# baycom/tfrec

Measured on AMD Instinct MI355X. Metric: IQ MSamples/s through demod+decode (batched streams), higher is better.
Workload: dtype int32+f32+f64

## Files before the change

### tfrec_amd/csrc/chains2.hip

```cpp
#include <stdlib.h>

#include <algorithm>

#include "decoder_dev.h"
#include <type_traits>
#include "whb_chain_asm.h"

namespace tfrec {

constexpr int kSpecLbi = -(1 << 30);

__device__ __forceinline__ int whb_hook_perturb(const WinTables &T)
{
#ifdef TFREC_AMD_EXPERIMENTS
	return T.whb_test_perturb;
#else
	return 0;
#endif
}
__device__ __forceinline__ int whb_hook_force_fail(const WinTables &T)
{
#ifdef TFREC_AMD_EXPERIMENTS
	return T.whb_force_fail;
#else
	return 0;
#endif
}

__device__ __forceinline__ int tfa1_decay(int m) { return m - (int)(((uint32_t)m + 19u) / 20u); }

constexpr int kStatTfa1Scalar = 7, kStatTfa2Scalar = 8, kStatTfa1Vector = 9, kStatTfa2Vector = 10;
struct GroupStats {
	int scalar, vector;
};
__device__ __forceinline__ void stat_flush(const WinTables &T, const GroupStats &g, int slot_scalar, int slot_vector)
{
#if !defined(TFREC_AMD_COOPSTAT) && !defined(TFREC_AMD_VECSTAT) && !defined(TFREC_AMD_PROFILE_WHB)
	if ((threadIdx.x & 63) == 0) {
		if (g.scalar)
			atomicAdd(&T.stats[slot_scalar], (unsigned long long)g.scalar);
#ifdef TFREC_AMD_EXPERIMENTS
		if (g.vector)
			atomicAdd(&T.stats[slot_vector], (unsigned long long)g.vector);
#endif
	}
#endif
}

__device__ __forceinline__ int rebase_lbi(int lbi, int from_block, int to_block)
{
	return lbi ? lbi - kIndexSpan * (to_block - from_block) : 0;
}

struct BitWriter {
	uint32_t *base;
	uint32_t acc;
	int n;
	uint32_t pend;
	int pend_idx;
	__device__ __forceinline__ void put(int bit)
	{
		acc |= (uint32_t)bit << (n & 31);
		n++;
		if ((n & 31) == 0) {
			if (pend_idx >= 0)
				base[pend_idx] = pend;
			pend = acc;
			pend_idx = (n >> 5) - 1;
			acc = 0;
		}
	}
	__device__ __forceinline__ void put_bits(uint32_t v, int cnt)
	{
		const int sh = n & 31;
		const unsigned long long a = (unsigned long long)acc | ((unsigned long long)v << sh);
		n += cnt;
		if (sh + cnt >= 32) {
			if (pend_idx >= 0)
				base[pend_idx] = pend;
			pend = (uint32_t)a;
			pend_idx = (n >> 5) - 1;
			acc = (uint32_t)(a >> 32);
		} else {
			acc = (uint32_t)a;
		}
	}
	__device__ __forceinline__ void chunk_end()
	{
		const int idx = pend_idx >= 0 ? pend_idx : (n >> 5);
		base[idx] = pend_idx >= 0 ? pend : acc;
		pend_idx = -1;
	}
	__device__ __forceinline__ void finish()
	{
		chunk_end();
		if (n & 31)
			base[n >> 5] = acc;
	}
};

#include "windows.h"

#include "biquad.h"

#include "slicers.h"

#include "coop_slicer.h"

#include "whb_commit.h"

#include "whb_demod.h"

#include "whb_check.h"

#include "decode.h"

hipError_t launch_fmdev(hipStream_t st, const uint32_t *dec, size_t dec_stride, const unsigned long long *mask,
			size_t mask_stride, const uint32_t *prevdec, int16_t *fmdev, size_t fmdev_stride, EventBuf *eb,
			int n_streams, int n_blocks, int wmax, double flag_eps);

hipError_t launch_pipeline(const PipeCtl &P, const uint32_t *dec, size_t dec_stride, const unsigned long long *mask,
			   size_t mask_stride, const int16_t *fmdev, size_t fmdev_stride, int n_streams, int n_blocks,
			   long long sample_base, const ChainLaunch &L, const WinTables &T, int16_t *ld16, int32_t *dev32,
			   tfrec_amd_event *events, EventBuf *eb, uint32_t flags)
{
	auto mark = [&](int k, hipStream_t s_) {
		if (P.tev)
			(void)hipEventRecord(P.tev[k], s_);
	};
	hipError_t e = hipSuccess;
#define TRY(x)                          \
	do {                            \
		if ((e = (x)) != hipSuccess) \
			return e;       \
	} while (0)
	if (L.n_active == 0) {
		for (int k = 0; k < 3; k++)
			TRY(hipEventRecord(P.done[k], k == 0 ? P.cs : (k == 1 ? P.aux : P.t1)));
		return hipSuccess;
	}
	constexpr int lanes = 64;
	constexpr int head_chunks = 64;
	dim3 block(64);
	dim3 grid((n_streams + lanes - 1) / lanes, L.n_active);
	const int win_blocks = std::min(16384, (int)(((size_t)n_streams * n_blocks * 2 + lanes - 1) / lanes));
	const int seg_blocks = std::min(16384, (int)(((size_t)L.n_active * n_streams * ((size_t)n_blocks * (kBlockDec / 32) / kSegSlots + 4) +
						       lanes - 1) / lanes));
	const int repair_blocks = std::min(seg_blocks, std::max(256, seg_blocks / 8));
	const int spec_blocks = std::min(seg_blocks, std::max(256, seg_blocks / 5));
	const int long_window = (size_t)n_streams * L.n_active >= 1024 ? kLongWindow : kLongWindow / 2;
	const int coop_blocks = std::min(32768, std::max(1, (int)std::min<size_t>((size_t)L.n_active * n_streams *
								((size_t)n_blocks * kBlockDec / (size_t)long_window + 1), 1u << 30)));
	const int dec_blocks = std::min(16384, std::max(1, win_blocks));
	bool has_whb = false, has_tfa2 = false, has_tfa1 = false;
	for (int a = 0; a < L.n_active; a++) {
		has_whb = has_whb || L.params[a].kind == 2;
		has_tfa2 = has_tfa2 || L.params[a].kind == 1;
		has_tfa1 = has_tfa1 || L.params[a].kind == 0;
	}
// ... 147 lines not shown
```

### tfrec_amd/csrc/whb_check.h

```cpp
#pragma once

#ifndef TFREC_AMD_CHK_STREAMS
#define TFREC_AMD_CHK_STREAMS 32
#endif
constexpr int kChkStreams = TFREC_AMD_CHK_STREAMS;
constexpr int kChkProducers = 2;
constexpr int kChkPerProducer = kChkStreams / kChkProducers;
static_assert(kChkStreams <= 64 && kChkStreams % kChkProducers == 0, "a lane per stream, the streams split evenly");
constexpr int kChkPairRow = 64 * 4 + 4;
constexpr int kChkDevRow = 64 + 4;
struct ChkBuf {
	uint32_t pair[kChkStreams * kChkPairRow];
	uint32_t dev[kChkStreams * kChkDevRow];
};
constexpr size_t kChkLdsBytes = 2 * sizeof(ChkBuf);

__global__ __launch_bounds__(64 * (1 + kChkProducers)) void whb_chain_kernel(int n_streams, ChainLaunch L, int a, WinTables T)
{
	extern __shared__ __attribute__((aligned(16))) uint8_t chk_lds[];
	ChkBuf *const buf = reinterpret_cast<ChkBuf *>(chk_lds);
	const int wave = (int)threadIdx.x >> 6, ln = (int)threadIdx.x & 63;
	const int s0 = (int)blockIdx.x * kChkStreams;
	const ChainParams &p = L.params[a];
	const double a1 = p.iir_avg.a1, a2 = p.iir_avg.a2, bh = 0.5 * p.iir_avg.b0;
	const int my_s = s0 + ln;
	const bool my_on = ln < kChkStreams && my_s < n_streams;
	const int my_rounds = my_on ? T.whbdense_n[my_s] >> 6 : 0;
	int rmax = my_rounds;
#pragma unroll
	for (int o = 32; o >= 1; o >>= 1) {
		const int other = __shfl_xor(rmax, o, 64);
		rmax = other > rmax ? other : rmax;
	}
	rmax = __builtin_amdgcn_readfirstlane(rmax);
	if (rmax == 0)
		return;
	if (wave == 0) {
		double y1 = 0.0, y2 = 0.0;
		if (my_on) {
			const WhbExact st = T.whbx[my_s];
			y1 = st.y1;
			y2 = st.y2;
		}
		unsigned long long *const xbits = T.whbxbits + (size_t)(my_on ? my_s : 0) * T.whbx_stride;
		double2 *const xsnap = T.whbxsnap + (size_t)(my_on ? my_s : 0) * T.whbx_stride;
		__syncthreads();
		for (int r = 0; r < rmax; r++) {
			if (r < my_rounds) {
				const ChkBuf &b = buf[r & 1];
				const double2 *prow = reinterpret_cast<const double2 *>(b.pair + ln * kChkPairRow);
				const uint4 *drow = reinterpret_cast<const uint4 *>(b.dev + ln * kChkDevRow);
				uint32_t acc[2] = { 0u, 0u };
				double2 pq[2][8];
				uint4 dq[2][2];
				auto fetch = [&](int h, int g8) {
#pragma unroll
					for (int j = 0; j < 8; j++)
						pq[h][j] = prow[8 * g8 + j];
					dq[h][0] = drow[2 * g8];
					dq[h][1] = drow[2 * g8 + 1];
				};
				fetch(0, 0);
#pragma unroll
				for (int g8 = 0; g8 < 8; g8++) {
					const int h = g8 & 1;
					if (g8 + 1 < 8)
						fetch(h ^ 1, g8 + 1);
					const int dv[8] = { (int)dq[h][0].x, (int)dq[h][0].y, (int)dq[h][0].z, (int)dq[h][0].w,
							    (int)dq[h][1].x, (int)dq[h][1].y, (int)dq[h][1].z, (int)dq[h][1].w };
#pragma unroll
					for (int j = 0; j < 8; j++) {
						const double P = pq[h][j].x, B2 = pq[h][j].y;
						const double y = ((B2 + a1 * y1) + P) + a2 * y2;
						y2 = y1;
						y1 = y;
						const int yi = (int)y;
						asm("v_cmp_lt_i32 vcc, %1, %2\n\tv_addc_co_u32 %0, vcc, %0, %0, vcc" : "+v"(acc[g8 >> 2]) : "v"(dv[j]), "v"(yi) : "vcc");
					}
				}
				xbits[r] = (unsigned long long)__brev(acc[0]) | ((unsigned long long)__brev(acc[1]) << 32);
				xsnap[r] = make_double2(y1, y2);
			}
			__syncthreads();
		}
	} else {
		const int q0 = (wave - 1) * kChkPerProducer;
		int rounds[kChkPerProducer], h1[kChkPerProducer], h2[kChkPerProducer];
		const int32_t *row[kChkPerProducer];
#pragma unroll
		for (int q = 0; q < kChkPerProducer; q++) {
			const int s = s0 + q0 + q;
			const bool on = s < n_streams;
			rounds[q] = __builtin_amdgcn_readlane(my_rounds, (q0 + q) & 63);
			row[q] = T.whbdense + (size_t)(on ? s : 0) * T.whbdense_stride;
			const WhbExact st = T.whbx[on ? s : 0];
			h1[q] = __builtin_amdgcn_readfirstlane(st.fd1);
			h2[q] = __builtin_amdgcn_readfirstlane(st.fd2);
		}
		int cur[kChkPerProducer], nxt[kChkPerProducer];
#pragma unroll
		for (int q = 0; q < kChkPerProducer; q++) {
			cur[q] = rounds[q] > 0 ? row[q][ln] : 0;
			nxt[q] = rounds[q] > 1 ? row[q][64 + ln] : 0;
		}
		auto lay_out = [&](ChkBuf &b, int r) {
#pragma unroll
			for (int q = 0; q < kChkPerProducer; q++) {
				if (r < rounds[q]) {
					const int d0 = cur[q];
					const int s1 = __builtin_amdgcn_update_dpp(0, d0, 0x138, 0xf, 0xf, false);
					const int d1 = ln == 0 ? h1[q] : s1;
					const int s2 = __builtin_amdgcn_update_dpp(0, d1, 0x138, 0xf, 0xf, false);
					const int d2 = ln == 0 ? h2[q] : s2;
					const double t0 = bh * (double)d0, t1 = bh * (double)d1, t2 = bh * (double)d2;
					const double P = __builtin_fma(2.0, t1, t0);
					*reinterpret_cast<double2 *>(b.pair + (q0 + q) * kChkPairRow + 4 * ln) = make_double2(P, t2);
					b.dev[(q0 + q) * kChkDevRow + ln] = (uint32_t)d0;
					h1[q] = __builtin_amdgcn_readlane(d0, 63);
					h2[q] = __builtin_amdgcn_readlane(d0, 62);
				}
			}
		};
		lay_out(buf[0], 0);
		__syncthreads();
		for (int r = 0; r < rmax; r++) {
			int far[kChkPerProducer];
#pragma unroll
			for (int q = 0; q < kChkPerProducer; q++)
				far[q] = r + 2 < rounds[q] ? row[q][64 * (r + 2) + ln] : 0;
#pragma unroll
			for (int q = 0; q < kChkPerProducer; q++)
				cur[q] = nxt[q];
			if (r + 1 < rmax)
				lay_out(buf[(r + 1) & 1], r + 1);
#pragma unroll
			for (int q = 0; q < kChkPerProducer; q++)
				nxt[q] = far[q];
			__syncthreads();
		}
	}
}

constexpr int kChkLockCap = 256;
__global__ __launch_bounds__(64) void whb_check_kernel(int n_streams, ChainLaunch L, int a, WinTables T, int *__restrict__ carry_io)
{
	__shared__ int lk_pos[kChkLockCap], lk_avgf[kChkLockCap];
	__shared__ uint32_t lk_meta[kChkLockCap];
	const int s = (int)blockIdx.x, ln = (int)threadIdx.x;
	if (s >= n_streams)
		return;
	const ChainParams &p = L.params[a];
	const double a1 = p.iir_avg.a1, a2 = p.iir_avg.a2, bh = 0.5 * p.iir_avg.b0;
	const int N = T.whbdense_n[s], R = N >> 6;
	const int32_t *dense = T.whbdense + (size_t)s * T.whbdense_stride;
	const unsigned long long *xbits = T.whbxbits + (size_t)s * T.whbx_stride;
	const double2 *xsnap = T.whbxsnap + (size_t)s * T.whbx_stride;
	const WhbExact st0 = T.whbx[s];
	const int tp_ = whb_hook_perturb(T);
	const int tol = tp_ > 1 ? tp_ : (tp_ < -1 ? -tp_ : 1);
	auto input = [&](int pos) -> int { return pos >= 0 ? dense[pos] : (pos == -1 ? st0.fd1 : st0.fd2); };
	auto run = [&](int rr, int cnt, double &y1, double &y2, unsigned long long &bits) {
		const int p0 = 64 * rr;
		if (rr == 0) {
			y1 = st0.y1;
			y2 = st0.y2;
		} else {
			const double2 sn = xsnap[rr - 1];
			y1 = sn.x;
			y2 = sn.y;
		}
		double t1 = bh * (double)input(p0 - 1), t2 = bh * (double)input(p0 - 2);
		bits = 0ull;
		for (int k = 0; k < cnt; k++) {
			const int d = dense[p0 + k];
			const double t0 = bh * (double)d;
			const double P = __builtin_fma(2.0, t1, t0);
			const double y = ((t2 + a1 * y1) + P) + a2 * y2;
			bits |= (unsigned long long)(d < (int)y ? 1u : 0u) << k;
			y2 = y1;
			y1 = y;
			t2 = t1;
			t1 = t0;
		}
	};
	double yf1 = 0.0, yf2 = 0.0;
	unsigned long long tailbits = 0ull;
	if (ln == 0)
		run(R, N & 63, yf1, yf2, tailbits);
	tailbits = __shfl(tailbits, 0, 64);
	auto word = [&](int i) -> unsigned long long { return i < R ? xbits[i] : (i == R ? tailbits : 0ull); };
	const uint4 *recrow = reinterpret_cast<const uint4 *>(T.whbrec + (size_t)s * T.whbrec_stride);
	int carry = carry_io[s];
	const int carry_in = carry;
	bool bad = false;
	int cbase = 0, nlocks = 0;
	bool ended = false;
	int last_delta = 0;
	bool have_last = false, last_closed = false;
	auto do_locks = [&]() {
		for (int b0 = 0; b0 < nlocks; b0 += 64) {
			const int i = b0 + ln;
			const bool on = i < nlocks;
			double y1 = 0.0, y2 = 0.0;
			unsigned long long bits;
			const int pos = on ? lk_pos[i] : 0;
			run(pos >> 6, on ? (pos & 63) + 1 : 0, y1, y2, bits);
			const uint32_t meta = on ? lk_meta[i] : 0u;
			const int delta = (int)y1 - (on ? lk_avgf[i] : 0);
			const bool b = on && (delta > tol || delta < -tol || (delta != 0 && (meta & kWhbRecAmb)));
			bad = bad || __ballot(b) != 0ull;
			const int nb = nlocks - b0 < 64 ? nlocks - b0 : 64;
			last_delta = __shfl(delta, nb - 1, 64);
			last_closed = (__shfl((int)meta, nb - 1, 64) & (int)kWhbRecClosed) != 0;
			have_last = true;
		}
		nlocks = 0;
	};
	for (int v0 = 0; !ended; v0 += 64) {
		const int vi = v0 + ln < T.whbrec_stride - 1 ? v0 + ln : T.whbrec_stride - 1;
		const uint4 rec = recrow[vi];
		const uint32_t meta = rec.z;
		const unsigned long long endm = __ballot(meta == kWhbRecEnd);
		const int nrec = endm ? __builtin_ctzll(endm) : 64;
		ended = endm != 0ull || v0 + 64 + 64 > T.whbrec_stride;
		const bool on = ln < nrec;
		const bool pseudo = on && (meta & kWhbRecPseudo) != 0u;
		const bool normal = on && !pseudo;
		const int nv = normal ? (int)((meta >> kWhbRecNvShift) & 63u) + 1 : 0;
		int inc = nv;
#pragma unroll
		for (int o = 1; o < 64; o <<= 1) {
			const int up = __shfl_up(inc, o, 64);
			inc += ln >= o ? up : 0;
		}
		const int pos0 = cbase + inc - nv;
		cbase += __shfl(inc, 63, 64);
		if (pseudo) {
			if (v0 + ln == 0) {
				bad = bad || (carry != 0 && (meta & kWhbRecAmb));
				if (meta & kWhbRecClosed)
					carry = 0;
			} else {
				bad = true;
			}
		}
		if (normal) {
			const int w = pos0 >> 6, sh = pos0 & 63;
			const unsigned long long lo = word(w) >> sh, hi = sh ? word(w + 1) << (64 - sh) : 0ull;
			const unsigned long long vm = nv >= 64 ? ~0ull : (1ull << nv) - 1ull;
			const unsigned long long below = ((unsigned long long)rec.y << 32) | rec.x;
			bad = bad || (((lo | hi) ^ below) & vm) != 0ull || pos0 + nv > N;
		}
		carry = __shfl(carry, 0, 64);
		const bool lock = normal && (meta & kWhbRecLock) != 0u;
		const unsigned long long lm = __ballot(lock);
		if (lm) {
			if (nlocks + 64 > kChkLockCap)
				do_locks();
			if (lock) {
				const int i = nlocks + __builtin_popcountll(lm & ((1ull << ln) - 1ull));
				lk_pos[i] = pos0 + nv - 1;
				lk_avgf[i] = (int)rec.w;
				lk_meta[i] = meta;
			}
			nlocks += __builtin_popcountll(lm);
			__syncthreads();
		}
	}
	if (nlocks)
		do_locks();
	bad = __ballot(bad) != 0ull || cbase != N;
	if (have_last)
		carry = last_closed ? 0 : last_delta;
	if (ln == 0) {
		WhbExact st = st0;
		st.carry = carry_in;
		st.pad_ = 0;
		T.whbx0[s] = st;
		bad = bad || T.whbseen[s] != T.whbgen[s];
		if (whb_hook_force_fail(T) > 0 && (s + T.whb_submit_seq) % whb_hook_force_fail(T) == 0)
			bad = true;
		st.y1 = yf1;
		st.y2 = yf2;
		st.fd1 = input(N - 1);
		st.fd2 = input(N - 2);
		st.carry = st.pad_ = 0;
		T.whbx[s] = st;
		carry_io[s] = bad ? 0 : carry;
		T.whbfail[s] = bad ? 1 : 0;
	}
}

// ... 1 lines not shown
```

Measured before the change: 303,600.

## Move IIR threshold decisions to producer waves and hand-schedule consumer recurrence in asm

The consumer wave now runs only the serial f64 IIR recurrence through a generated inline-asm block with explicit LDS read lookahead, and writes each y value back to LDS. The compare-against-sample bit packing and the xbits/xsnap global stores move to the producer waves, which use ballots one round behind. The intent is to shorten the serial critical path on the consumer wave by taking the integer conversion, compare and global stores off it. In exchange, LDS traffic grows with the y row, the asm hardcodes VGPRs 64-105, and the producers gain a decide stage and an extra drain step.

```diff
diff --git a/tfrec_amd/csrc/chains2.hip b/tfrec_amd/csrc/chains2.hip
--- a/tfrec_amd/csrc/chains2.hip
+++ b/tfrec_amd/csrc/chains2.hip
@@ -5,6 +5,7 @@
 #include "decoder_dev.h"
 #include <type_traits>
 #include "whb_chain_asm.h"
+#include "whb_consumer_asm.h"
 
 namespace tfrec {
 
diff --git a/tfrec_amd/csrc/gen_whb_consumer.py b/tfrec_amd/csrc/gen_whb_consumer.py
--- /dev/null
+++ b/tfrec_amd/csrc/gen_whb_consumer.py
@@ -0,0 +1,85 @@
+#!/usr/bin/env python3
+import os
+import sys
+
+BASE = 64
+LOOKAHEAD = 8
+N_IN = 64
+REG_PAIR = [BASE + 4 * i for i in range(LOOKAHEAD)]
+REG_T = BASE + 4 * LOOKAHEAD
+REG_Q = [REG_T + 2, REG_T + 4]
+REG_Y01 = [REG_T + 6, REG_T + 8]
+LAST = REG_T + 9
+
+
+def vp(r):
+    return "v[%d:%d]" % (r, r + 1)
+
+
+def y(k):
+    k &= 3
+    return vp(REG_Y01[k]) if k < 2 else "%%[Y%d]" % k
+
+
+def pair_p(k):
+    return vp(REG_PAIR[k % LOOKAHEAD])
+
+
+def pair_b(k):
+    return vp(REG_PAIR[k % LOOKAHEAD] + 2)
+
+
+def block():
+    L = []
+    lgkm = []
+
+    def read(k):
+        L.append("ds_read_b128 v[%d:%d], %%[prow] offset:%d" % (REG_PAIR[k % LOOKAHEAD], REG_PAIR[k % LOOKAHEAD] + 3, 16 * k))
+        lgkm.append(("r", k))
+
+    def write(k):
+        L.append("ds_write2_b64 %%[yrow], %s, %s offset0:%d offset1:%d" % (y(k), y(k + 1), k, k + 1))
+        lgkm.append(("w", k))
+
+    def wait_for(op):
+        n = len(lgkm) - 1 - lgkm.index(op)
+        L.append("s_waitcnt lgkmcnt(%d)" % min(n, 15))
+
+    for k in range(LOOKAHEAD):
+        read(k)
+    L.append("v_mul_f64 %s, %%[a2], %s" % (vp(REG_Q[0]), y(-2)))
+    for k in range(N_IN):
+        L.append("v_mul_f64 %s, %%[a1], %s" % (vp(REG_T), y(k - 1)))
+        if k + 1 < N_IN:
+            L.append("v_mul_f64 %s, %%[a2], %s" % (vp(REG_Q[(k + 1) & 1]), y(k - 1)))
+        if k % 2 == 0:
+            wait_for(("r", k + 1))
+        L.append("v_add_f64 %s, %s, %s" % (vp(REG_T), pair_b(k), vp(REG_T)))
+        if k % 2 == 0 and k >= 2:
+            write(k - 2)
+        L.append("v_add_f64 %s, %s, %s" % (vp(REG_T), vp(REG_T), pair_p(k)))
+        if k + LOOKAHEAD < N_IN:
+            read(k + LOOKAHEAD)
+        L.append("v_add_f64 %s, %s, %s" % (y(k), vp(REG_T), vp(REG_Q[k & 1])))
+    write(N_IN - 2)
+    L.append("s_waitcnt lgkmcnt(0)")
+    return L
+
+
+def header():
+    out = ["// GENERATED by tfrec_amd/csrc/gen_whb_consumer.py -- do not edit (see the generator for the design).", "#pragma once",
+           "#define TFREC_WHB_CONSUMER_ASM \\"]
+    out.append(" \\\n".join('\t"%s\\n"' % x for x in block()))
+    out.append("#define TFREC_WHB_CONSUMER_CLOBBERS %s" % ", ".join('"v%d"' % r for r in range(BASE, LAST + 1)))
+    return "\n".join(out) + "\n"
+
+
+def main():
+    out = sys.argv[1] if len(sys.argv) > 1 else os.path.join(os.path.dirname(os.path.abspath(__file__)), "whb_consumer_asm.h")
+    with open(out, "w") as f:
+        f.write(header())
+    print("wrote", out)
+
+
+if __name__ == "__main__":
+    main()
diff --git a/tfrec_amd/csrc/whb_check.h b/tfrec_amd/csrc/whb_check.h
--- a/tfrec_amd/csrc/whb_check.h
+++ b/tfrec_amd/csrc/whb_check.h
@@ -8,12 +8,18 @@
 constexpr int kChkPerProducer = kChkStreams / kChkProducers;
 static_assert(kChkStreams <= 64 && kChkStreams % kChkProducers == 0, "a lane per stream, the streams split evenly");
 constexpr int kChkPairRow = 64 * 4 + 4;
-constexpr int kChkDevRow = 64 + 4;
+constexpr int kChkYRow = 64 * 2 + 4;
 struct ChkBuf {
 	uint32_t pair[kChkStreams * kChkPairRow];
-	uint32_t dev[kChkStreams * kChkDevRow];
+	uint32_t y[kChkStreams * kChkYRow];
 };
 constexpr size_t kChkLdsBytes = 2 * sizeof(ChkBuf);
+static_assert(kChkLdsBytes <= 160 * 1024, "one workgroup per CU");
+
+__device__ inline uint32_t chk_lds_addr(const uint32_t *p)
+{
+	return (uint32_t)(uintptr_t)(const __attribute__((address_space(3))) uint32_t *)p;
+}
 
 __global__ __launch_bounds__(64 * (1 + kChkProducers)) void whb_chain_kernel(int n_streams, ChainLaunch L, int a, WinTables T)
 {
@@ -42,44 +48,16 @@
 			y1 = st.y1;
 			y2 = st.y2;
 		}
-		unsigned long long *const xbits = T.whbxbits + (size_t)(my_on ? my_s : 0) * T.whbx_stride;
-		double2 *const xsnap = T.whbxsnap + (size_t)(my_on ? my_s : 0) * T.whbx_stride;
+		const int row = ln < kChkStreams ? ln : 0;
 		__syncthreads();
 		for (int r = 0; r < rmax; r++) {
 			if (r < my_rounds) {
 				const ChkBuf &b = buf[r & 1];
-				const double2 *prow = reinterpret_cast<const double2 *>(b.pair + ln * kChkPairRow);
-				const uint4 *drow = reinterpret_cast<const uint4 *>(b.dev + ln * kChkDevRow);
-				uint32_t acc[2] = { 0u, 0u };
-				double2 pq[2][8];
-				uint4 dq[2][2];
-				auto fetch = [&](int h, int g8) {
-#pragma unroll
-					for (int j = 0; j < 8; j++)
-						pq[h][j] = prow[8 * g8 + j];
-					dq[h][0] = drow[2 * g8];
-					dq[h][1] = drow[2 * g8 + 1];
-				};
-				fetch(0, 0);
-#pragma unroll
-				for (int g8 = 0; g8 < 8; g8++) {
-					const int h = g8 & 1;
-					if (g8 + 1 < 8)
-						fetch(h ^ 1, g8 + 1);
-					const int dv[8] = { (int)dq[h][0].x, (int)dq[h][0].y, (int)dq[h][0].z, (int)dq[h][0].w,
-							    (int)dq[h][1].x, (int)dq[h][1].y, (int)dq[h][1].z, (int)dq[h][1].w };
-#pragma unroll
-					for (int j = 0; j < 8; j++) {
-						const double P = pq[h][j].x, B2 = pq[h][j].y;
-						const double y = ((B2 + a1 * y1) + P) + a2 * y2;
-						y2 = y1;
-						y1 = y;
-						const int yi = (int)y;
-						asm("v_cmp_lt_i32 vcc, %1, %2\n\tv_addc_co_u32 %0, vcc, %0, %0, vcc" : "+v"(acc[g8 >> 2]) : "v"(dv[j]), "v"(yi) : "vcc");
-					}
-				}
-				xbits[r] = (unsigned long long)__brev(acc[0]) | ((unsigned long long)__brev(acc[1]) << 32);
-				xsnap[r] = make_double2(y1, y2);
+				const uint32_t prow = chk_lds_addr(b.pair + row * kChkPairRow), yrow = chk_lds_addr(b.y + row * kChkYRow);
+				asm volatile(TFREC_WHB_CONSUMER_ASM
+					     : [Y2] "+v"(y2), [Y3] "+v"(y1)
+					     : [prow] "v"(prow), [yrow] "v"(yrow), [a1] "s"(a1), [a2] "s"(a2)
+					     : "memory", TFREC_WHB_CONSUMER_CLOBBERS);
 			}
 			__syncthreads();
 		}
@@ -97,7 +75,13 @@
 			h1[q] = __builtin_amdgcn_readfirstlane(st.fd1);
 			h2[q] = __builtin_amdgcn_readfirstlane(st.fd2);
 		}
-		int cur[kChkPerProducer], nxt[kChkPerProducer];
+		const int st_q = ln < kChkPerProducer ? ln : 0;
+		const int st_rounds_all = __shfl(my_rounds, q0 + st_q, 64);
+		const int st_rounds = ln < kChkPerProducer ? st_rounds_all : 0;
+		const size_t st_off = (size_t)(s0 + q0 + st_q < n_streams ? s0 + q0 + st_q : 0) * T.whbx_stride;
+		unsigned long long *const xbits = T.whbxbits + st_off;
+		double2 *const xsnap = T.whbxsnap + st_off;
+		int prev[kChkPerProducer], cur[kChkPerProducer], nxt[kChkPerProducer];
 #pragma unroll
 		for (int q = 0; q < kChkPerProducer; q++) {
 			cur[q] = rounds[q] > 0 ? row[q][ln] : 0;
@@ -115,22 +99,45 @@
 					const double t0 = bh * (double)d0, t1 = bh * (double)d1, t2 = bh * (double)d2;
 					const double P = __builtin_fma(2.0, t1, t0);
 					*reinterpret_cast<double2 *>(b.pair + (q0 + q) * kChkPairRow + 4 * ln) = make_double2(P, t2);
-					b.dev[(q0 + q) * kChkDevRow + ln] = (uint32_t)d0;
 					h1[q] = __builtin_amdgcn_readlane(d0, 63);
 					h2[q] = __builtin_amdgcn_readlane(d0, 62);
 				}
+			}
+		};
+		auto decide = [&](const ChkBuf &b, int r) {
+			double y[kChkPerProducer];
+#pragma unroll
+			for (int q = 0; q < kChkPerProducer; q++)
+				y[q] = reinterpret_cast<const double *>(b.y + (q0 + q) * kChkYRow)[ln];
+			const double2 yt = reinterpret_cast<const double2 *>(b.y + (q0 + st_q) * kChkYRow)[31];
+			uint32_t lo = 0u, hi = 0u;
+#pragma unroll
+			for (int q = 0; q < kChkPerProducer; q++) {
+				const unsigned long long m = __builtin_amdgcn_ballot_w64(prev[q] < (int)y[q]);
+				asm volatile("s_nop 4\n\tv_writelane_b32 %0, %2, %4\n\tv_writelane_b32 %1, %3, %4"
+					     : "+v"(lo), "+v"(hi)
+					     : "s"((uint32_t)m), "s"((uint32_t)(m >> 32)), "i"(q));
+			}
+			if (r < st_rounds) {
+				xbits[r] = ((unsigned long long)hi << 32) | lo;
+				xsnap[r] = make_double2(yt.y, yt.x);
 			}
 		};
 		lay_out(buf[0], 0);
 		__syncthreads();
 		for (int r = 0; r < rmax; r++) {
+			__builtin_amdgcn_s_waitcnt(0x0f70);
+			if (r > 0)
+				decide(buf[(r - 1) & 1], r - 1);
 			int far[kChkPerProducer];
 #pragma unroll
 			for (int q = 0; q < kChkPerProducer; q++)
 				far[q] = r + 2 < rounds[q] ? row[q][64 * (r + 2) + ln] : 0;
 #pragma unroll
-			for (int q = 0; q < kChkPerProducer; q++)
+			for (int q = 0; q < kChkPerProducer; q++) {
+				prev[q] = cur[q];
 				cur[q] = nxt[q];
+			}
 			if (r + 1 < rmax)
 				lay_out(buf[(r + 1) & 1], r + 1);
 #pragma unroll
@@ -138,6 +145,7 @@
 				nxt[q] = far[q];
 			__syncthreads();
 		}
+		decide(buf[(rmax - 1) & 1], rmax - 1);
 	}
 }
 
diff --git a/tfrec_amd/csrc/whb_consumer_asm.h b/tfrec_amd/csrc/whb_consumer_asm.h
--- /dev/null
+++ b/tfrec_amd/csrc/whb_consumer_asm.h
@@ -0,0 +1,452 @@
+#pragma once
+#define TFREC_WHB_CONSUMER_ASM \
+	"ds_read_b128 v[64:67], %[prow] offset:0\n" \
+	"ds_read_b128 v[68:71], %[prow] offset:16\n" \
+	"ds_read_b128 v[72:75], %[prow] offset:32\n" \
+	"ds_read_b128 v[76:79], %[prow] offset:48\n" \
+	"ds_read_b128 v[80:83], %[prow] offset:64\n" \
+	"ds_read_b128 v[84:87], %[prow] offset:80\n" \
+	"ds_read_b128 v[88:91], %[prow] offset:96\n" \
+	"ds_read_b128 v[92:95], %[prow] offset:112\n" \
+	"v_mul_f64 v[98:99], %[a2], %[Y2]\n" \
+	"v_mul_f64 v[96:97], %[a1], %[Y3]\n" \
+	"v_mul_f64 v[100:101], %[a2], %[Y3]\n" \
+	"s_waitcnt lgkmcnt(6)\n" \
+	"v_add_f64 v[96:97], v[66:67], v[96:97]\n" \
+	"v_add_f64 v[96:97], v[96:97], v[64:65]\n" \
+	"ds_read_b128 v[64:67], %[prow] offset:128\n" \
+	"v_add_f64 v[102:103], v[96:97], v[98:99]\n" \
+	"v_mul_f64 v[96:97], %[a1], v[102:103]\n" \
+	"v_mul_f64 v[98:99], %[a2], v[102:103]\n" \
+	"v_add_f64 v[96:97], v[70:71], v[96:97]\n" \
+	"v_add_f64 v[96:97], v[96:97], v[68:69]\n" \
+	"ds_read_b128 v[68:71], %[prow] offset:144\n" \
+	"v_add_f64 v[104:105], v[96:97], v[100:101]\n" \
+	"v_mul_f64 v[96:97], %[a1], v[104:105]\n" \
+	"v_mul_f64 v[100:101], %[a2], v[104:105]\n" \
+	"s_waitcnt lgkmcnt(6)\n" \
+	"v_add_f64 v[96:97], v[74:75], v[96:97]\n" \
+	"ds_write2_b64 %[yrow], v[102:103], v[104:105] offset0:0 offset1:1\n" \
+	"v_add_f64 v[96:97], v[96:97], v[72:73]\n" \
+	"ds_read_b128 v[72:75], %[prow] offset:160\n" \
+	"v_add_f64 %[Y2], v[96:97], v[98:99]\n" \
+	"v_mul_f64 v[96:97], %[a1], %[Y2]\n" \
+	"v_mul_f64 v[98:99], %[a2], %[Y2]\n" \
+	"v_add_f64 v[96:97], v[78:79], v[96:97]\n" \
+	"v_add_f64 v[96:97], v[96:97], v[76:77]\n" \
+	"ds_read_b128 v[76:79], %[prow] offset:176\n" \
+	"v_add_f64 %[Y3], v[96:97], v[100:101]\n" \
+	"v_mul_f64 v[96:97], %[a1], %[Y3]\n" \
+	"v_mul_f64 v[100:101], %[a2], %[Y3]\n" \
+	"s_waitcnt lgkmcnt(7)\n" \
+	"v_add_f64 v[96:97], v[82:83], v[96:97]\n" \
+	"ds_write2_b64 %[yrow], %[Y2], %[Y3] offset0:2 offset1:3\n" \
+	"v_add_f64 v[96:97], v[96:97], v[80:81]\n" \
+	"ds_read_b128 v[80:83], %[prow] offset:192\n" \
+	"v_add_f64 v[102:103], v[96:97], v[98:99]\n" \
+	"v_mul_f64 v[96:97], %[a1], v[102:103]\n" \
+	"v_mul_f64 v[98:99], %[a2], v[102:103]\n" \
+	"v_add_f64 v[96:97], v[86:87], v[96:97]\n" \
+	"v_add_f64 v[96:97], v[96:97], v[84:85]\n" \
+	"ds_read_b128 v[84:87], %[prow] offset:208\n" \
+	"v_add_f64 v[104:105], v[96:97], v[100:101]\n" \
+	"v_mul_f64 v[96:97], %[a1], v[104:105]\n" \
+	"v_mul_f64 v[100:101], %[a2], v[104:105]\n" \
+	"s_waitcnt lgkmcnt(8)\n" \
+	"v_add_f64 v[96:97], v[90:91], v[96:97]\n" \
+	"ds_write2_b64 %[yrow], v[102:103], v[104:105] offset0:4 offset1:5\n" \
+	"v_add_f64 v[96:97], v[96:97], v[88:89]\n" \
+	"ds_read_b128 v[88:91], %[prow] offset:224\n" \
+	"v_add_f64 %[Y2], v[96:97], v[98:99]\n" \
+	"v_mul_f64 v[96:97], %[a1], %[Y2]\n" \
+	"v_mul_f64 v[98:99], %[a2], %[Y2]\n" \
+	"v_add_f64 v[96:97], v[94:95], v[96:97]\n" \
+	"v_add_f64 v[96:97], v[96:97], v[92:93]\n" \
+	"ds_read_b128 v[92:95], %[prow] offset:240\n" \
+	"v_add_f64 %[Y3], v[96:97], v[100:101]\n" \
+	"v_mul_f64 v[96:97], %[a1], %[Y3]\n" \
+	"v_mul_f64 v[100:101], %[a2], %[Y3]\n" \
+	"s_waitcnt lgkmcnt(9)\n" \
+	"v_add_f64 v[96:97], v[66:67], v[96:97]\n" \
+	"ds_write2_b64 %[yrow], %[Y2], %[Y3] offset0:6 offset1:7\n" \
+	"v_add_f64 v[96:97], v[96:97], v[64:65]\n" \
+	"ds_read_b128 v[64:67], %[prow] offset:256\n" \
+	"v_add_f64 v[102:103], v[96:97], v[98:99]\n" \
+	"v_mul_f64 v[96:97], %[a1], v[102:103]\n" \
+	"v_mul_f64 v[98:99], %[a2], v[102:103]\n" \
+	"v_add_f64 v[96:97], v[70:71], v[96:97]\n" \
+	"v_add_f64 v[96:97], v[96:97], v[68:69]\n" \
+	"ds_read_b128 v[68:71], %[prow] offset:272\n" \
+	"v_add_f64 v[104:105], v[96:97], v[100:101]\n" \
+	"v_mul_f64 v[96:97], %[a1], v[104:105]\n" \
+	"v_mul_f64 v[100:101], %[a2], v[104:105]\n" \
+	"s_waitcnt lgkmcnt(9)\n" \
+	"v_add_f64 v[96:97], v[74:75], v[96:97]\n" \
+	"ds_write2_b64 %[yrow], v[102:103], v[104:105] offset0:8 offset1:9\n" \
+	"v_add_f64 v[96:97], v[96:97], v[72:73]\n" \
+	"ds_read_b128 v[72:75], %[prow] offset:288\n" \
+	"v_add_f64 %[Y2], v[96:97], v[98:99]\n" \
+	"v_mul_f64 v[96:97], %[a1], %[Y2]\n" \
+	"v_mul_f64 v[98:99], %[a2], %[Y2]\n" \
+	"v_add_f64 v[96:97], v[78:79], v[96:97]\n" \
+	"v_add_f64 v[96:97], v[96:97], v[76:77]\n" \
+	"ds_read_b128 v[76:79], %[prow] offset:304\n" \
+	"v_add_f64 %[Y3], v[96:97], v[100:101]\n" \
+	"v_mul_f64 v[96:97], %[a1], %[Y3]\n" \
+	"v_mul_f64 v[100:101], %[a2], %[Y3]\n" \
+	"s_waitcnt lgkmcnt(9)\n" \
+	"v_add_f64 v[96:97], v[82:83], v[96:97]\n" \
+	"ds_write2_b64 %[yrow], %[Y2], %[Y3] offset0:10 offset1:11\n" \
+	"v_add_f64 v[96:97], v[96:97], v[80:81]\n" \
+	"ds_read_b128 v[80:83], %[prow] offset:320\n" \
+	"v_add_f64 v[102:103], v[96:97], v[98:99]\n" \
+	"v_mul_f64 v[96:97], %[a1], v[102:103]\n" \
+	"v_mul_f64 v[98:99], %[a2], v[102:103]\n" \
+	"v_add_f64 v[96:97], v[86:87], v[96:97]\n" \
+	"v_add_f64 v[96:97], v[96:97], v[84:85]\n" \
+	"ds_read_b128 v[84:87], %[prow] offset:336\n" \
+	"v_add_f64 v[104:105], v[96:97], v[100:101]\n" \
+	"v_mul_f64 v[96:97], %[a1], v[104:105]\n" \
+	"v_mul_f64 v[100:101], %[a2], v[104:105]\n" \
+	"s_waitcnt lgkmcnt(9)\n" \
+	"v_add_f64 v[96:97], v[90:91], v[96:97]\n" \
+	"ds_write2_b64 %[yrow], v[102:103], v[104:105] offset0:12 offset1:13\n" \
+	"v_add_f64 v[96:97], v[96:97], v[88:89]\n" \
+	"ds_read_b128 v[88:91], %[prow] offset:352\n" \
+	"v_add_f64 %[Y2], v[96:97], v[98:99]\n" \
+	"v_mul_f64 v[96:97], %[a1], %[Y2]\n" \
+	"v_mul_f64 v[98:99], %[a2], %[Y2]\n" \
+	"v_add_f64 v[96:97], v[94:95], v[96:97]\n" \
+	"v_add_f64 v[96:97], v[96:97], v[92:93]\n" \
+	"ds_read_b128 v[92:95], %[prow] offset:368\n" \
+	"v_add_f64 %[Y3], v[96:97], v[100:101]\n" \
+	"v_mul_f64 v[96:97], %[a1], %[Y3]\n" \
+	"v_mul_f64 v[100:101], %[a2], %[Y3]\n" \
+	"s_waitcnt lgkmcnt(9)\n" \
+	"v_add_f64 v[96:97], v[66:67], v[96:97]\n" \
+	"ds_write2_b64 %[yrow], %[Y2], %[Y3] offset0:14 offset1:15\n" \
+	"v_add_f64 v[96:97], v[96:97], v[64:65]\n" \
+	"ds_read_b128 v[64:67], %[prow] offset:384\n" \
+	"v_add_f64 v[102:103], v[96:97], v[98:99]\n" \
+	"v_mul_f64 v[96:97], %[a1], v[102:103]\n" \
+	"v_mul_f64 v[98:99], %[a2], v[102:103]\n" \
+	"v_add_f64 v[96:97], v[70:71], v[96:97]\n" \
+	"v_add_f64 v[96:97], v[96:97], v[68:69]\n" \
+	"ds_read_b128 v[68:71], %[prow] offset:400\n" \
+	"v_add_f64 v[104:105], v[96:97], v[100:101]\n" \
+	"v_mul_f64 v[96:97], %[a1], v[104:105]\n" \
+	"v_mul_f64 v[100:101], %[a2], v[104:105]\n" \
+	"s_waitcnt lgkmcnt(9)\n" \
+	"v_add_f64 v[96:97], v[74:75], v[96:97]\n" \
+	"ds_write2_b64 %[yrow], v[102:103], v[104:105] offset0:16 offset1:17\n" \
+	"v_add_f64 v[96:97], v[96:97], v[72:73]\n" \
+	"ds_read_b128 v[72:75], %[prow] offset:416\n" \
+	"v_add_f64 %[Y2], v[96:97], v[98:99]\n" \
+	"v_mul_f64 v[96:97], %[a1], %[Y2]\n" \
+	"v_mul_f64 v[98:99], %[a2], %[Y2]\n" \
+	"v_add_f64 v[96:97], v[78:79], v[96:97]\n" \
+	"v_add_f64 v[96:97], v[96:97], v[76:77]\n" \
+	"ds_read_b128 v[76:79], %[prow] offset:432\n" \
+	"v_add_f64 %[Y3], v[96:97], v[100:101]\n" \
+	"v_mul_f64 v[96:97], %[a1], %[Y3]\n" \
+	"v_mul_f64 v[100:101], %[a2], %[Y3]\n" \
+	"s_waitcnt lgkmcnt(9)\n" \
+	"v_add_f64 v[96:97], v[82:83], v[96:97]\n" \
+	"ds_write2_b64 %[yrow], %[Y2], %[Y3] offset0:18 offset1:19\n" \
+	"v_add_f64 v[96:97], v[96:97], v[80:81]\n" \
+	"ds_read_b128 v[80:83], %[prow] offset:448\n" \
+	"v_add_f64 v[102:103], v[96:97], v[98:99]\n" \
+	"v_mul_f64 v[96:97], %[a1], v[102:103]\n" \
+	"v_mul_f64 v[98:99], %[a2], v[102:103]\n" \
+	"v_add_f64 v[96:97], v[86:87], v[96:97]\n" \
+	"v_add_f64 v[96:97], v[96:97], v[84:85]\n" \
+	"ds_read_b128 v[84:87], %[prow] offset:464\n" \
+	"v_add_f64 v[104:105], v[96:97], v[100:101]\n" \
+	"v_mul_f64 v[96:97], %[a1], v[104:105]\n" \
+	"v_mul_f64 v[100:101], %[a2], v[104:105]\n" \
+	"s_waitcnt lgkmcnt(9)\n" \
+	"v_add_f64 v[96:97], v[90:91], v[96:97]\n" \
+	"ds_write2_b64 %[yrow], v[102:103], v[104:105] offset0:20 offset1:21\n" \
+	"v_add_f64 v[96:97], v[96:97], v[88:89]\n" \
+	"ds_read_b128 v[88:91], %[prow] offset:480\n" \
+	"v_add_f64 %[Y2], v[96:97], v[98:99]\n" \
+	"v_mul_f64 v[96:97], %[a1], %[Y2]\n" \
+	"v_mul_f64 v[98:99], %[a2], %[Y2]\n" \
+	"v_add_f64 v[96:97], v[94:95], v[96:97]\n" \
+	"v_add_f64 v[96:97], v[96:97], v[92:93]\n" \
+	"ds_read_b128 v[92:95], %[prow] offset:496\n" \
+	"v_add_f64 %[Y3], v[96:97], v[100:101]\n" \
+	"v_mul_f64 v[96:97], %[a1], %[Y3]\n" \
+	"v_mul_f64 v[100:101], %[a2], %[Y3]\n" \
+	"s_waitcnt lgkmcnt(9)\n" \
+	"v_add_f64 v[96:97], v[66:67], v[96:97]\n" \
+	"ds_write2_b64 %[yrow], %[Y2], %[Y3] offset0:22 offset1:23\n" \
+	"v_add_f64 v[96:97], v[96:97], v[64:65]\n" \
+	"ds_read_b128 v[64:67], %[prow] offset:512\n" \
+	"v_add_f64 v[102:103], v[96:97], v[98:99]\n" \
+	"v_mul_f64 v[96:97], %[a1], v[102:103]\n" \
+	"v_mul_f64 v[98:99], %[a2], v[102:103]\n" \
+	"v_add_f64 v[96:97], v[70:71], v[96:97]\n" \
+	"v_add_f64 v[96:97], v[96:97], v[68:69]\n" \
+	"ds_read_b128 v[68:71], %[prow] offset:528\n" \
+	"v_add_f64 v[104:105], v[96:97], v[100:101]\n" \
+	"v_mul_f64 v[96:97], %[a1], v[104:105]\n" \
+	"v_mul_f64 v[100:101], %[a2], v[104:105]\n" \
+	"s_waitcnt lgkmcnt(9)\n" \
+	"v_add_f64 v[96:97], v[74:75], v[96:97]\n" \
+	"ds_write2_b64 %[yrow], v[102:103], v[104:105] offset0:24 offset1:25\n" \
+	"v_add_f64 v[96:97], v[96:97], v[72:73]\n" \
+	"ds_read_b128 v[72:75], %[prow] offset:544\n" \
+	"v_add_f64 %[Y2], v[96:97], v[98:99]\n" \
+	"v_mul_f64 v[96:97], %[a1], %[Y2]\n" \
+	"v_mul_f64 v[98:99], %[a2], %[Y2]\n" \
+	"v_add_f64 v[96:97], v[78:79], v[96:97]\n" \
+	"v_add_f64 v[96:97], v[96:97], v[76:77]\n" \
+	"ds_read_b128 v[76:79], %[prow] offset:560\n" \
+	"v_add_f64 %[Y3], v[96:97], v[100:101]\n" \
+	"v_mul_f64 v[96:97], %[a1], %[Y3]\n" \
+	"v_mul_f64 v[100:101], %[a2], %[Y3]\n" \
+	"s_waitcnt lgkmcnt(9)\n" \
+	"v_add_f64 v[96:97], v[82:83], v[96:97]\n" \
+	"ds_write2_b64 %[yrow], %[Y2], %[Y3] offset0:26 offset1:27\n" \
+	"v_add_f64 v[96:97], v[96:97], v[80:81]\n" \
+	"ds_read_b128 v[80:83], %[prow] offset:576\n" \
+	"v_add_f64 v[102:103], v[96:97], v[98:99]\n" \
+	"v_mul_f64 v[96:97], %[a1], v[102:103]\n" \
+	"v_mul_f64 v[98:99], %[a2], v[102:103]\n" \
+	"v_add_f64 v[96:97], v[86:87], v[96:97]\n" \
+	"v_add_f64 v[96:97], v[96:97], v[84:85]\n" \
+	"ds_read_b128 v[84:87], %[prow] offset:592\n" \
+	"v_add_f64 v[104:105], v[96:97], v[100:101]\n" \
+	"v_mul_f64 v[96:97], %[a1], v[104:105]\n" \
+	"v_mul_f64 v[100:101], %[a2], v[104:105]\n" \
+	"s_waitcnt lgkmcnt(9)\n" \
+	"v_add_f64 v[96:97], v[90:91], v[96:97]\n" \
+	"ds_write2_b64 %[yrow], v[102:103], v[104:105] offset0:28 offset1:29\n" \
+	"v_add_f64 v[96:97], v[96:97], v[88:89]\n" \
+	"ds_read_b128 v[88:91], %[prow] offset:608\n" \
+	"v_add_f64 %[Y2], v[96:97], v[98:99]\n" \
+	"v_mul_f64 v[96:97], %[a1], %[Y2]\n" \
+	"v_mul_f64 v[98:99], %[a2], %[Y2]\n" \
+	"v_add_f64 v[96:97], v[94:95], v[96:97]\n" \
+	"v_add_f64 v[96:97], v[96:97], v[92:93]\n" \
+	"ds_read_b128 v[92:95], %[prow] offset:624\n" \
+	"v_add_f64 %[Y3], v[96:97], v[100:101]\n" \
+	"v_mul_f64 v[96:97], %[a1], %[Y3]\n" \
+	"v_mul_f64 v[100:101], %[a2], %[Y3]\n" \
+	"s_waitcnt lgkmcnt(9)\n" \
+	"v_add_f64 v[96:97], v[66:67], v[96:97]\n" \
+	"ds_write2_b64 %[yrow], %[Y2], %[Y3] offset0:30 offset1:31\n" \
+	"v_add_f64 v[96:97], v[96:97], v[64:65]\n" \
+	"ds_read_b128 v[64:67], %[prow] offset:640\n" \
+	"v_add_f64 v[102:103], v[96:97], v[98:99]\n" \
+	"v_mul_f64 v[96:97], %[a1], v[102:103]\n" \
+	"v_mul_f64 v[98:99], %[a2], v[102:103]\n" \
+	"v_add_f64 v[96:97], v[70:71], v[96:97]\n" \
+	"v_add_f64 v[96:97], v[96:97], v[68:69]\n" \
+	"ds_read_b128 v[68:71], %[prow] offset:656\n" \
+	"v_add_f64 v[104:105], v[96:97], v[100:101]\n" \
+	"v_mul_f64 v[96:97], %[a1], v[104:105]\n" \
+	"v_mul_f64 v[100:101], %[a2], v[104:105]\n" \
+	"s_waitcnt lgkmcnt(9)\n" \
+	"v_add_f64 v[96:97], v[74:75], v[96:97]\n" \
+	"ds_write2_b64 %[yrow], v[102:103], v[104:105] offset0:32 offset1:33\n" \
+	"v_add_f64 v[96:97], v[96:97], v[72:73]\n" \
+	"ds_read_b128 v[72:75], %[prow] offset:672\n" \
+	"v_add_f64 %[Y2], v[96:97], v[98:99]\n" \
+	"v_mul_f64 v[96:97], %[a1], %[Y2]\n" \
+	"v_mul_f64 v[98:99], %[a2], %[Y2]\n" \
+	"v_add_f64 v[96:97], v[78:79], v[96:97]\n" \
+	"v_add_f64 v[96:97], v[96:97], v[76:77]\n" \
+	"ds_read_b128 v[76:79], %[prow] offset:688\n" \
+	"v_add_f64 %[Y3], v[96:97], v[100:101]\n" \
+	"v_mul_f64 v[96:97], %[a1], %[Y3]\n" \
+	"v_mul_f64 v[100:101], %[a2], %[Y3]\n" \
+	"s_waitcnt lgkmcnt(9)\n" \
+	"v_add_f64 v[96:97], v[82:83], v[96:97]\n" \
+	"ds_write2_b64 %[yrow], %[Y2], %[Y3] offset0:34 offset1:35\n" \
+	"v_add_f64 v[96:97], v[96:97], v[80:81]\n" \
+	"ds_read_b128 v[80:83], %[prow] offset:704\n" \
+	"v_add_f64 v[102:103], v[96:97], v[98:99]\n" \
+	"v_mul_f64 v[96:97], %[a1], v[102:103]\n" \
+	"v_mul_f64 v[98:99], %[a2], v[102:103]\n" \
+	"v_add_f64 v[96:97], v[86:87], v[96:97]\n" \
+	"v_add_f64 v[96:97], v[96:97], v[84:85]\n" \
+	"ds_read_b128 v[84:87], %[prow] offset:720\n" \
+	"v_add_f64 v[104:105], v[96:97], v[100:101]\n" \
+	"v_mul_f64 v[96:97], %[a1], v[104:105]\n" \
+	"v_mul_f64 v[100:101], %[a2], v[104:105]\n" \
+	"s_waitcnt lgkmcnt(9)\n" \
+	"v_add_f64 v[96:97], v[90:91], v[96:97]\n" \
+	"ds_write2_b64 %[yrow], v[102:103], v[104:105] offset0:36 offset1:37\n" \
+	"v_add_f64 v[96:97], v[96:97], v[88:89]\n" \
+	"ds_read_b128 v[88:91], %[prow] offset:736\n" \
+	"v_add_f64 %[Y2], v[96:97], v[98:99]\n" \
+	"v_mul_f64 v[96:97], %[a1], %[Y2]\n" \
+	"v_mul_f64 v[98:99], %[a2], %[Y2]\n" \
+	"v_add_f64 v[96:97], v[94:95], v[96:97]\n" \
+	"v_add_f64 v[96:97], v[96:97], v[92:93]\n" \
+	"ds_read_b128 v[92:95], %[prow] offset:752\n" \
+	"v_add_f64 %[Y3], v[96:97], v[100:101]\n" \
+	"v_mul_f64 v[96:97], %[a1], %[Y3]\n" \
+	"v_mul_f64 v[100:101], %[a2], %[Y3]\n" \
+	"s_waitcnt lgkmcnt(9)\n" \
+	"v_add_f64 v[96:97], v[66:67], v[96:97]\n" \
+	"ds_write2_b64 %[yrow], %[Y2], %[Y3] offset0:38 offset1:39\n" \
+	"v_add_f64 v[96:97], v[96:97], v[64:65]\n" \
+	"ds_read_b128 v[64:67], %[prow] offset:768\n" \
+	"v_add_f64 v[102:103], v[96:97], v[98:99]\n" \
+	"v_mul_f64 v[96:97], %[a1], v[102:103]\n" \
+	"v_mul_f64 v[98:99], %[a2], v[102:103]\n" \
+	"v_add_f64 v[96:97], v[70:71], v[96:97]\n" \
+	"v_add_f64 v[96:97], v[96:97], v[68:69]\n" \
+	"ds_read_b128 v[68:71], %[prow] offset:784\n" \
+	"v_add_f64 v[104:105], v[96:97], v[100:101]\n" \
+	"v_mul_f64 v[96:97], %[a1], v[104:105]\n" \
+	"v_mul_f64 v[100:101], %[a2], v[104:105]\n" \
+	"s_waitcnt lgkmcnt(9)\n" \
+	"v_add_f64 v[96:97], v[74:75], v[96:97]\n" \
+	"ds_write2_b64 %[yrow], v[102:103], v[104:105] offset0:40 offset1:41\n" \
+	"v_add_f64 v[96:97], v[96:97], v[72:73]\n" \
+	"ds_read_b128 v[72:75], %[prow] offset:800\n" \
+	"v_add_f64 %[Y2], v[96:97], v[98:99]\n" \
+	"v_mul_f64 v[96:97], %[a1], %[Y2]\n" \
+	"v_mul_f64 v[98:99], %[a2], %[Y2]\n" \
+	"v_add_f64 v[96:97], v[78:79], v[96:97]\n" \
+	"v_add_f64 v[96:97], v[96:97], v[76:77]\n" \
+	"ds_read_b128 v[76:79], %[prow] offset:816\n" \
+	"v_add_f64 %[Y3], v[96:97], v[100:101]\n" \
+	"v_mul_f64 v[96:97], %[a1], %[Y3]\n" \
+	"v_mul_f64 v[100:101], %[a2], %[Y3]\n" \
+	"s_waitcnt lgkmcnt(9)\n" \
+	"v_add_f64 v[96:97], v[82:83], v[96:97]\n" \
+	"ds_write2_b64 %[yrow], %[Y2], %[Y3] offset0:42 offset1:43\n" \
+	"v_add_f64 v[96:97], v[96:97], v[80:81]\n" \
+	"ds_read_b128 v[80:83], %[prow] offset:832\n" \
+	"v_add_f64 v[102:103], v[96:97], v[98:99]\n" \
+	"v_mul_f64 v[96:97], %[a1], v[102:103]\n" \
+	"v_mul_f64 v[98:99], %[a2], v[102:103]\n" \
+	"v_add_f64 v[96:97], v[86:87], v[96:97]\n" \
+	"v_add_f64 v[96:97], v[96:97], v[84:85]\n" \
+	"ds_read_b128 v[84:87], %[prow] offset:848\n" \
+	"v_add_f64 v[104:105], v[96:97], v[100:101]\n" \
+	"v_mul_f64 v[96:97], %[a1], v[104:105]\n" \
+	"v_mul_f64 v[100:101], %[a2], v[104:105]\n" \
+	"s_waitcnt lgkmcnt(9)\n" \
+	"v_add_f64 v[96:97], v[90:91], v[96:97]\n" \
+	"ds_write2_b64 %[yrow], v[102:103], v[104:105] offset0:44 offset1:45\n" \
+	"v_add_f64 v[96:97], v[96:97], v[88:89]\n" \
+	"ds_read_b128 v[88:91], %[prow] offset:864\n" \
+	"v_add_f64 %[Y2], v[96:97], v[98:99]\n" \
+	"v_mul_f64 v[96:97], %[a1], %[Y2]\n" \
+	"v_mul_f64 v[98:99], %[a2], %[Y2]\n" \
+	"v_add_f64 v[96:97], v[94:95], v[96:97]\n" \
+	"v_add_f64 v[96:97], v[96:97], v[92:93]\n" \
+	"ds_read_b128 v[92:95], %[prow] offset:880\n" \
+	"v_add_f64 %[Y3], v[96:97], v[100:101]\n" \
+	"v_mul_f64 v[96:97], %[a1], %[Y3]\n" \
+	"v_mul_f64 v[100:101], %[a2], %[Y3]\n" \
+	"s_waitcnt lgkmcnt(9)\n" \
+	"v_add_f64 v[96:97], v[66:67], v[96:97]\n" \
+	"ds_write2_b64 %[yrow], %[Y2], %[Y3] offset0:46 offset1:47\n" \
+	"v_add_f64 v[96:97], v[96:97], v[64:65]\n" \
+	"ds_read_b128 v[64:67], %[prow] offset:896\n" \
+	"v_add_f64 v[102:103], v[96:97], v[98:99]\n" \
+	"v_mul_f64 v[96:97], %[a1], v[102:103]\n" \
+	"v_mul_f64 v[98:99], %[a2], v[102:103]\n" \
+	"v_add_f64 v[96:97], v[70:71], v[96:97]\n" \
+	"v_add_f64 v[96:97], v[96:97], v[68:69]\n" \
+	"ds_read_b128 v[68:71], %[prow] offset:912\n" \
+	"v_add_f64 v[104:105], v[96:97], v[100:101]\n" \
+	"v_mul_f64 v[96:97], %[a1], v[104:105]\n" \
+	"v_mul_f64 v[100:101], %[a2], v[104:105]\n" \
+	"s_waitcnt lgkmcnt(9)\n" \
+	"v_add_f64 v[96:97], v[74:75], v[96:97]\n" \
+	"ds_write2_b64 %[yrow], v[102:103], v[104:105] offset0:48 offset1:49\n" \
+	"v_add_f64 v[96:97], v[96:97], v[72:73]\n" \
+	"ds_read_b128 v[72:75], %[prow] offset:928\n" \
+	"v_add_f64 %[Y2], v[96:97], v[98:99]\n" \
+	"v_mul_f64 v[96:97], %[a1], %[Y2]\n" \
+	"v_mul_f64 v[98:99], %[a2], %[Y2]\n" \
+	"v_add_f64 v[96:97], v[78:79], v[96:97]\n" \
+	"v_add_f64 v[96:97], v[96:97], v[76:77]\n" \
+	"ds_read_b128 v[76:79], %[prow] offset:944\n" \
+	"v_add_f64 %[Y3], v[96:97], v[100:101]\n" \
+	"v_mul_f64 v[96:97], %[a1], %[Y3]\n" \
+	"v_mul_f64 v[100:101], %[a2], %[Y3]\n" \
+	"s_waitcnt lgkmcnt(9)\n" \
+	"v_add_f64 v[96:97], v[82:83], v[96:97]\n" \
+	"ds_write2_b64 %[yrow], %[Y2], %[Y3] offset0:50 offset1:51\n" \
+	"v_add_f64 v[96:97], v[96:97], v[80:81]\n" \
+	"ds_read_b128 v[80:83], %[prow] offset:960\n" \
+	"v_add_f64 v[102:103], v[96:97], v[98:99]\n" \
+	"v_mul_f64 v[96:97], %[a1], v[102:103]\n" \
+	"v_mul_f64 v[98:99], %[a2], v[102:103]\n" \
+	"v_add_f64 v[96:97], v[86:87], v[96:97]\n" \
+	"v_add_f64 v[96:97], v[96:97], v[84:85]\n" \
+	"ds_read_b128 v[84:87], %[prow] offset:976\n" \
+	"v_add_f64 v[104:105], v[96:97], v[100:101]\n" \
+	"v_mul_f64 v[96:97], %[a1], v[104:105]\n" \
+	"v_mul_f64 v[100:101], %[a2], v[104:105]\n" \
+	"s_waitcnt lgkmcnt(9)\n" \
+	"v_add_f64 v[96:97], v[90:91], v[96:97]\n" \
+	"ds_write2_b64 %[yrow], v[102:103], v[104:105] offset0:52 offset1:53\n" \
+	"v_add_f64 v[96:97], v[96:97], v[88:89]\n" \
+	"ds_read_b128 v[88:91], %[prow] offset:992\n" \
+	"v_add_f64 %[Y2], v[96:97], v[98:99]\n" \
+	"v_mul_f64 v[96:97], %[a1], %[Y2]\n" \
+	"v_mul_f64 v[98:99], %[a2], %[Y2]\n" \
+	"v_add_f64 v[96:97], v[94:95], v[96:97]\n" \
+	"v_add_f64 v[96:97], v[96:97], v[92:93]\n" \
+	"ds_read_b128 v[92:95], %[prow] offset:1008\n" \
+	"v_add_f64 %[Y3], v[96:97], v[100:101]\n" \
+	"v_mul_f64 v[96:97], %[a1], %[Y3]\n" \
+	"v_mul_f64 v[100:101], %[a2], %[Y3]\n" \
+	"s_waitcnt lgkmcnt(9)\n" \
+	"v_add_f64 v[96:97], v[66:67], v[96:97]\n" \
+	"ds_write2_b64 %[yrow], %[Y2], %[Y3] offset0:54 offset1:55\n" \
+	"v_add_f64 v[96:97], v[96:97], v[64:65]\n" \
+	"v_add_f64 v[102:103], v[96:97], v[98:99]\n" \
+	"v_mul_f64 v[96:97], %[a1], v[102:103]\n" \
+	"v_mul_f64 v[98:99], %[a2], v[102:103]\n" \
+	"v_add_f64 v[96:97], v[70:71], v[96:97]\n" \
+	"v_add_f64 v[96:97], v[96:97], v[68:69]\n" \
+	"v_add_f64 v[104:105], v[96:97], v[100:101]\n" \
+	"v_mul_f64 v[96:97], %[a1], v[104:105]\n" \
+	"v_mul_f64 v[100:101], %[a2], v[104:105]\n" \
+	"s_waitcnt lgkmcnt(7)\n" \
+	"v_add_f64 v[96:97], v[74:75], v[96:97]\n" \
+	"ds_write2_b64 %[yrow], v[102:103], v[104:105] offset0:56 offset1:57\n" \
+	"v_add_f64 v[96:97], v[96:97], v[72:73]\n" \
+	"v_add_f64 %[Y2], v[96:97], v[98:99]\n" \
+	"v_mul_f64 v[96:97], %[a1], %[Y2]\n" \
+	"v_mul_f64 v[98:99], %[a2], %[Y2]\n" \
+	"v_add_f64 v[96:97], v[78:79], v[96:97]\n" \
+	"v_add_f64 v[96:97], v[96:97], v[76:77]\n" \
+	"v_add_f64 %[Y3], v[96:97], v[100:101]\n" \
+	"v_mul_f64 v[96:97], %[a1], %[Y3]\n" \
+	"v_mul_f64 v[100:101], %[a2], %[Y3]\n" \
+	"s_waitcnt lgkmcnt(5)\n" \
+	"v_add_f64 v[96:97], v[82:83], v[96:97]\n" \
+	"ds_write2_b64 %[yrow], %[Y2], %[Y3] offset0:58 offset1:59\n" \
+	"v_add_f64 v[96:97], v[96:97], v[80:81]\n" \
+	"v_add_f64 v[102:103], v[96:97], v[98:99]\n" \
+	"v_mul_f64 v[96:97], %[a1], v[102:103]\n" \
+	"v_mul_f64 v[98:99], %[a2], v[102:103]\n" \
+	"v_add_f64 v[96:97], v[86:87], v[96:97]\n" \
+	"v_add_f64 v[96:97], v[96:97], v[84:85]\n" \
+	"v_add_f64 v[104:105], v[96:97], v[100:101]\n" \
+	"v_mul_f64 v[96:97], %[a1], v[104:105]\n" \
+	"v_mul_f64 v[100:101], %[a2], v[104:105]\n" \
+	"s_waitcnt lgkmcnt(3)\n" \
+	"v_add_f64 v[96:97], v[90:91], v[96:97]\n" \
+	"ds_write2_b64 %[yrow], v[102:103], v[104:105] offset0:60 offset1:61\n" \
+	"v_add_f64 v[96:97], v[96:97], v[88:89]\n" \
+	"v_add_f64 %[Y2], v[96:97], v[98:99]\n" \
+	"v_mul_f64 v[96:97], %[a1], %[Y2]\n" \
+	"v_add_f64 v[96:97], v[94:95], v[96:97]\n" \
+	"v_add_f64 v[96:97], v[96:97], v[92:93]\n" \
+	"v_add_f64 %[Y3], v[96:97], v[100:101]\n" \
+	"ds_write2_b64 %[yrow], %[Y2], %[Y3] offset0:62 offset1:63\n" \
+	"s_waitcnt lgkmcnt(0)\n"
+#define TFREC_WHB_CONSUMER_CLOBBERS "v64", "v65", "v66", "v67", "v68", "v69", "v70", "v71", "v72", "v73", "v74", "v75", "v76", "v77", "v78", "v79", "v80", "v81", "v82", "v83", "v84", "v85", "v86", "v87", "v88", "v89", "v90", "v91", "v92", "v93", "v94", "v95", "v96", "v97", "v98", "v99", "v100", "v101", "v102", "v103", "v104", "v105"
```

Measured after the change: 290,400 (median of 2 runs). 0.957x the previous value.
